# Maboroshi0327/MHAda-Style-Transfer

Hardware: AMD Instinct MI355X
Metric: stylized frames/sec (whole job) at 512x512 batch 8 fp32 [configs[1]] (higher is better)
Workload: dtype f32; 1 GPU; stylize 512x512 content+style, batch 8; resolution=512, batch_per_gpu=8, global_batch=8, compute_dtype=f32, parallelism=replicas x1

## Files before the change

mhada-style-transfer_amd/csrc/abi.hip:

```cpp
#include "common.h"

#include <mutex>
#include <stdlib.h>
#include <string.h>

namespace mhada {

static thread_local std::string g_last_error;

void set_error(const std::string& msg) { g_last_error = msg; }

int fail(const std::string& msg) {
  set_error(msg);
  return MHADA_ERR_ARG;
}

int check_launch(const char* what) {
  const hipError_t e = hipGetLastError();
  if (e != hipSuccess) {
    set_error(std::string(what) + ": " + hipGetErrorString(e));
    return MHADA_ERR_LAUNCH;
  }
  return MHADA_OK;
}

namespace {
struct Knob {
  const char* name;
  int Tuning::*field;
};
const Knob kKnobs[] = {
    {"attn_fixed_shift", &Tuning::attn_fixed_shift}, {"attn_waves", &Tuning::attn_waves},
    {"attn_tk", &Tuning::attn_tk},                   {"attn_prio", &Tuning::attn_prio},
    {"vit_attn_vec", &Tuning::vit_attn_vec},         {"out3_mfma", &Tuning::out3_mfma},
    {"out3_tile", &Tuning::out3_tile},               {"gemm_pp", &Tuning::gemm_pp},
    {"gemm_persist", &Tuning::gemm_persist},         {"gemm_pp128", &Tuning::gemm_pp128},
    {"gemm_ldsepi", &Tuning::gemm_ldsepi},           {"gemm_n64", &Tuning::gemm_n64},
    {"conv_c64", &Tuning::conv_c64},                 {"conv_dir", &Tuning::conv_dir},                 {"gemm_rinit", &Tuning::gemm_rinit},
    {"tn_skinny_lds", &Tuning::tn_skinny_lds},       {"train_dkv_dma", &Tuning::train_dkv_dma},
    {"wino_split3", &Tuning::wino_split3},           {"gemm_s3_order", &Tuning::gemm_s3_order},
    {"wino4", &Tuning::wino4},                       {"upsample_quad", &Tuning::upsample_quad},
    {"xknob", &Tuning::xknob},
};

Tuning g_tuning;
std::once_flag g_tuning_once;

void read_env_once() {
  std::call_once(g_tuning_once, [] {
    for (const Knob& k : kKnobs) {
      std::string env = "MHADA_";
      for (const char* c = k.name; *c; ++c) env += (char)(*c >= 'a' && *c <= 'z' ? *c - 32 : *c);
      if (const char* v = getenv(env.c_str())) g_tuning.*k.field = atoi(v);
    }
  });
}

bool valid(const char* name, int v) {
  if (!strcmp(name, "attn_waves")) return v == 0 || v == 4 || v == 8;
  if (!strcmp(name, "attn_tk")) return v == 64 || v == 128;
  if (!strcmp(name, "gemm_n64")) return v == 128 || v == 256;
  if (!strcmp(name, "xknob")) return v >= 0 && v < 16;
  return v == 0 || v == 1;
}
}

const Tuning& tuning() {
  read_env_once();
  return g_tuning;
}

}

extern "C" int mhada_abi_version(void) { return 18; }

extern "C" const char* mhada_last_error(void) { return mhada::g_last_error.c_str(); }

extern "C" int mhada_set_tuning(const char* name, int value) {
  using namespace mhada;
  read_env_once();
  if (!name) return fail("mhada_set_tuning: null name");
  for (const Knob& k : kKnobs) {
    if (!strcmp(k.name, name)) {
      if (!valid(name, value)) return fail(std::string("mhada_set_tuning: bad value for ") + name);
      g_tuning.*k.field = value;
      return MHADA_OK;
    }
  }
  return fail(std::string("mhada_set_tuning: unknown knob ") + name);
}

extern "C" int mhada_get_tuning(const char* name, int* value) {
  using namespace mhada;
  read_env_once();
  if (!name || !value) return fail("mhada_get_tuning: null argument");
  for (const Knob& k : kKnobs) {
    if (!strcmp(k.name, name)) {
      *value = g_tuning.*k.field;
      return MHADA_OK;
    }
  }
  return fail(std::string("mhada_get_tuning: unknown knob ") + name);
}
```

mhada-style-transfer_amd/csrc/common.h:

```cpp
#pragma once
#include <hip/hip_runtime.h>
#include <stdint.h>
#include <string>

#include "../../include/mhada_hip.h"

typedef __bf16 bf16;
typedef __bf16 bf16x8 __attribute__((ext_vector_type(8)));
typedef __bf16 bf16x4 __attribute__((ext_vector_type(4)));
typedef float f32x16 __attribute__((ext_vector_type(16)));
typedef float f32x4 __attribute__((ext_vector_type(4)));
typedef float f32x2 __attribute__((ext_vector_type(2)));

#define MHADA_DEV __device__ __forceinline__

namespace mhada {

void set_error(const std::string& msg);
int fail(const std::string& msg);
int check_launch(const char* what);

struct Tuning {
  int attn_fixed_shift = 1;
  int attn_waves = 0;
  int attn_tk = 128;
  int attn_prio = 1;
  int vit_attn_vec = 1;
  int out3_mfma = 1;
  int out3_tile = 1;
  int gemm_pp = 1;
  int gemm_persist = 1;
  int gemm_pp128 = 1;
  int gemm_ldsepi = 1;
  int gemm_n64 = 128;
  int conv_c64 = 1;
  int conv_dir = 1;
  int gemm_rinit = 1;
  int tn_skinny_lds = 1;
  int wino4 = 1;
  int wino_split3 = 1;
  int gemm_s3_order = 1;
  int train_dkv_dma = 1;
  int upsample_quad = 1;
  int xknob = 0;
};
const Tuning& tuning();

int conv3x3_c64(const void* x, const void* w, const float* bias, void* y, int B, int H, int W, bool up, int relu,
                hipStream_t s);
int conv3x3_dir(const void* x, const void* w, const float* bias, void* y, int B, int H, int W, int cin, int cout,
                int relu, hipStream_t s);

int vit_batch_attn_hd(const void* qkv, void* out, int dtype, int L, int ntok, int heads, int head_dim, hipStream_t s);

template <typename T> MHADA_DEV float to_f32(T x);
template <> MHADA_DEV float to_f32<float>(float x) { return x; }
template <> MHADA_DEV float to_f32<bf16>(bf16 x) { return (float)x; }

template <typename T> MHADA_DEV T from_f32(float x);
template <> MHADA_DEV float from_f32<float>(float x) { return x; }
template <> MHADA_DEV bf16 from_f32<bf16>(float x) { return (bf16)x; }

template <typename T> struct Vec16;
template <> struct Vec16<float> { typedef f32x4 type; static constexpr int N = 4; };
template <> struct Vec16<bf16> { typedef bf16x8 type; static constexpr int N = 8; };

MHADA_DEV float bilerp(float ly0, float ly1, float lx0, float lx1, float x00, float x01, float x10, float x11) {
  return fmaf(ly1, fmaf(lx0, x10, lx1 * x11), ly0 * fmaf(lx0, x00, lx1 * x01));
}

MHADA_DEV float wave_sum(float v) {
#pragma unroll
  for (int o = 32; o > 0; o >>= 1) v += __shfl_xor(v, o, 64);
  return v;
}
MHADA_DEV float wave_max(float v) {
#pragma unroll
  for (int o = 32; o > 0; o >>= 1) v = fmaxf(v, __shfl_xor(v, o, 64));
  return v;
}

MHADA_DEV int xcd_remap(int bid, int nblk) {
  const int q = nblk / 8, r = nblk % 8;
  const int xcd = bid % 8, k = bid / 8;
  return (xcd < r ? xcd * (q + 1) : r * (q + 1) + (xcd - r) * q) + k;
}

}
```

mhada-style-transfer_amd/csrc/wino.hip:

```cpp
#include "common.h"

#include <algorithm>
#include <utility>

#ifndef WINO_DBG
#define WINO_DBG 0
#endif
#ifndef WINO4_DBG
#define WINO4_DBG 0
#endif

namespace mhada {

namespace {
constexpr int kT = 8;
constexpr int kTT = kT * kT;
constexpr int kCO = 64;
constexpr int kCK = 8;
constexpr int kRP = 2 * kT + 2;
constexpr int kRaw = kRP * kRP;
constexpr int kRDma = (2 * kRaw + 63) / 64;
constexpr int kVS = 16 * kTT * kCK;
constexpr int kUS = 16 * kCO * kCK;
constexpr int kRS = kRDma * 64 * 4;

struct WinoP {
  const float* x;
  const float* u;
  const float* bias;
  float* y;
  const float* mask;
  int B, H, W, Cin, Cout, Ho, Wo, pad, zero, relu;
  long long ldc;
  int nbx, nby, nbn, nblk;
};

MHADA_DEV int reflect_clamp(int v, int n) {
  v = v < 0 ? -v : (v >= n ? 2 * n - 2 - v : v);
  return min(max(v, 0), n - 1);
}
MHADA_DEV int swz(int row, int half) { return row * 8 + ((half ^ ((row >> 3) & 1)) << 2); }
MHADA_DEV int rswz(int slot) { return slot ^ (((slot >> 3) & 1) << 1); }
MHADA_DEV int rswz4(int slot) { return slot ^ (((slot >> 4) & 1) << 1); }
MHADA_DEV void glds16(const float* src, float* lds) {
  __builtin_amdgcn_global_load_lds((const __attribute__((address_space(1))) void*)src,
                                   (__attribute__((address_space(3))) void*)lds, 16, 0, 0);
}


__global__ void __launch_bounds__(512, 1) wino_kernel(const WinoP p) {
  __shared__ __attribute__((aligned(16))) float lds[2 * (kVS + kUS + kRS)];
  auto sV = [&](int i) { return lds + i * kVS; };
  auto sU = [&](int i) { return lds + 2 * kVS + i * kUS; };
  auto sR = [&](int i) { return lds + 2 * (kVS + kUS) + i * kRS; };
  const int tid = threadIdx.x, lane = tid & 63, h = lane >> 5, r32 = lane & 31;
  const int wave = __builtin_amdgcn_readfirstlane(tid >> 6);
  const int e = wave >> 2, th = wave & 1, ch = (wave >> 1) & 1;

  int id = xcd_remap(blockIdx.x, p.nblk);
  const int nb = id % p.nbn;
  id /= p.nbn;
  const int bx = id % p.nbx;
  id /= p.nbx;
  const int by = id % p.nby;
  const int b = id / p.nby;
  const int co0 = nb * kCO;
  const int P = p.zero ? p.pad : 1;
  const int nck = p.Cin / kCK;

  int roff[2];
#pragma unroll
  for (int t = 0; t < 2; ++t) {
    const int slot = rswz(64 * (wave + 8 * t) + lane);
    const int px = min(slot >> 1, kRaw - 1);
    int iy = 2 * by * kT - P + px / kRP, ix = 2 * bx * kT - P + px % kRP;
    if (p.zero) {
      iy = min(max(iy, 0), p.H - 1);
      ix = min(max(ix, 0), p.W - 1);
    } else {
      iy = reflect_clamp(iy, p.H);
      ix = reflect_clamp(ix, p.W);
    }
    roff[t] = ((b * p.H + iy) * p.W + ix) * p.Cin + 4 * (slot & 1);
  }
  int uoff[4];
#pragma unroll
  for (int t = 0; t < 4; ++t) {
    const int slot = 64 * (4 * wave + t) + lane;
    const int xi = slot >> 7, row = (slot >> 1) & 63, sh = slot & 1;
    uoff[t] = (xi * p.Cout + co0 + row) * kCK + 4 * (sh ^ ((row >> 3) & 1));
  }
  const long long ustride = (long long)16 * p.Cout * kCK;
  auto dma = [&](int cu, float* su, int cr, float* sr) {
#if WINO_DBG & 2
    return;
#endif
    cu = min(cu, nck - 1);
    cr = min(cr, nck - 1);
    const float* uc = p.u + cu * ustride;
#pragma unroll
    for (int t = 0; t < 4; ++t) glds16(uc + uoff[t], su + (4 * wave + t) * 256);
    glds16(p.x + roff[0] + cr * kCK, sr + wave * 256);
    if (wave + 8 < kRDma) glds16(p.x + roff[1] + cr * kCK, sr + (wave + 8) * 256);
  };
  const int tc = tid & 7, tt = tid >> 3;
  int roffs[16];
#pragma unroll
  for (int i = 0; i < 4; ++i)
#pragma unroll
    for (int j = 0; j < 4; ++j) {
      const int pix = (2 * (tt >> 3) + i) * kRP + 2 * (tt & 7) + j;
      roffs[4 * i + j] = rswz(2 * pix + (tc >> 2)) * 4 + (tc & 3);
    }
  const int vdst = swz(tt, tc >> 2) + (tc & 3);
  unsigned zmask = 0;
  if (p.zero) {
    const int y0 = 2 * (by * kT + (tt >> 3)) - P, x0 = 2 * (bx * kT + (tt & 7)) - P;
#pragma unroll
    for (int i = 0; i < 4; ++i)
#pragma unroll
      for (int j = 0; j < 4; ++j)
        if (y0 + i < 0 || y0 + i >= p.H || x0 + j < 0 || x0 + j >= p.W) zmask |= 1u << (4 * i + j);
  }
  auto transform = [&](const float* sr, float* sv) {
#if WINO_DBG & 4
    return;
#endif
    float d[16];
#pragma unroll
    for (int i = 0; i < 4; ++i)
#pragma unroll
      for (int j = 0; j < 4; ++j) {
        const float v = sr[roffs[4 * i + j]];
        d[4 * i + j] = (zmask >> (4 * i + j)) & 1 ? 0.f : v;
      }
    float t[16];
#pragma unroll
    for (int j = 0; j < 4; ++j) {
      t[0 * 4 + j] = d[0 * 4 + j] - d[2 * 4 + j];
      t[1 * 4 + j] = d[1 * 4 + j] + d[2 * 4 + j];
      t[2 * 4 + j] = d[2 * 4 + j] - d[1 * 4 + j];
      t[3 * 4 + j] = d[1 * 4 + j] - d[3 * 4 + j];
    }
#pragma unroll
    for (int i = 0; i < 4; ++i) {
      sv[(4 * i + 0) * kTT * kCK + vdst] = t[4 * i + 0] - t[4 * i + 2];
      sv[(4 * i + 1) * kTT * kCK + vdst] = t[4 * i + 1] + t[4 * i + 2];
      sv[(4 * i + 2) * kTT * kCK + vdst] = t[4 * i + 2] - t[4 * i + 1];
      sv[(4 * i + 3) * kTT * kCK + vdst] = t[4 * i + 1] - t[4 * i + 3];
    }
  };

  f32x16 acc[8];
#pragma unroll
  for (int x = 0; x < 8; ++x)
#pragma unroll
    for (int q = 0; q < 16; ++q) acc[x][q] = 0.f;
  const int arow = swz(32 * th + r32, h) + 8 * e * (kTT * kCK), brow = swz(32 * ch + r32, h) + 8 * e * (kCO * kCK);
  auto mfmas = [&](const float* sv, const float* su) {
#if WINO_DBG & 1
    return;
#endif
#pragma unroll
    for (int x = 0; x < 8; ++x) {
      const f32x4 av = *reinterpret_cast<const f32x4*>(sv + x * (kTT * kCK) + arow);
      const f32x4 bv = *reinterpret_cast<const f32x4*>(su + x * (kCO * kCK) + brow);
#pragma unroll
      for (int s = 0; s < 4; ++s) acc[x] = __builtin_amdgcn_mfma_f32_32x32x2f32(av[s], bv[s], acc[x], 0, 0, 0);
    }
  };
  auto publish = [&]() {
    __builtin_amdgcn_sched_barrier(0);
    asm volatile("s_waitcnt vmcnt(0)" ::: "memory");
    __syncthreads();
  };

  dma(0, sU(0), 0, sR(0));
  dma(0, sU(0), 1, sR(1));
  publish();
  transform(sR(0), sV(0));
  __syncthreads();
  for (int k = 0; k < nck; ++k) {
    const int c = k & 1, n = c ^ 1;
    dma(k + 1, sU(n), k + 2, sR(c));
    mfmas(sV(c), sU(c));
    transform(sR(n), sV(n));
    publish();
  }

  float* ex = lds + (wave & 3) * (16 * 4 * 64) + lane;
  static_assert(4 * 16 * 4 * 64 <= 2 * kVS, "epilogue exchange must fit sV");
  if (e) {
#pragma unroll
    for (int r = 0; r < 16; ++r) {
      float m[2][2];
#pragma unroll
      for (int i = 0; i < 2; ++i) {
        const float m0 = acc[4 * i][r], m1 = acc[4 * i + 1][r], m2 = acc[4 * i + 2][r], m3 = acc[4 * i + 3][r];
        m[i][0] = m0 + m1 + m2;
        m[i][1] = m1 - m2 - m3;
      }
#pragma unroll
      for (int q = 0; q < 2; ++q) {
        ex[(r * 4 + 2 * q) * 64] = m[0][q];
        ex[(r * 4 + 2 * q + 1) * 64] = -m[0][q] - m[1][q];
      }
    }
  }
  __syncthreads();
  if (e) return;
  const int co = co0 + 32 * ch + r32;
  const float bias = p.bias ? p.bias[co] : 0.f;
#pragma unroll
  for (int r = 0; r < 16; ++r) {
    const int tile = 32 * th + (r & 3) + 8 * (r >> 2) + 4 * h;
    float m[2][2];
#pragma unroll
    for (int i = 0; i < 2; ++i) {
      const float m0 = acc[4 * i][r], m1 = acc[4 * i + 1][r], m2 = acc[4 * i + 2][r], m3 = acc[4 * i + 3][r];
      m[i][0] = m0 + m1 + m2;
      m[i][1] = m1 - m2 - m3;
    }
    const int oy0 = 2 * (by * kT + (tile >> 3)), ox0 = 2 * (bx * kT + (tile & 7));
#pragma unroll
    for (int q = 0; q < 2; ++q) {
      float y0 = m[0][q] + m[1][q] + ex[(r * 4 + 2 * q) * 64] + bias;
      float y1 = m[1][q] + ex[(r * 4 + 2 * q + 1) * 64] + bias;
      if (p.relu) {
        y0 = fmaxf(y0, 0.f);
        y1 = fmaxf(y1, 0.f);
      }
      const int ox = ox0 + q;
      if (ox < p.Wo) {
        const long long i0 = ((long long)(b * p.Ho + oy0) * p.Wo + ox) * p.ldc + co;
        const long long i1 = i0 + (long long)p.Wo * p.ldc;
        if (p.mask) {
          if (oy0 < p.Ho && !(p.mask[i0] > 0.f)) y0 = 0.f;
          if (oy0 + 1 < p.Ho && !(p.mask[i1] > 0.f)) y1 = 0.f;
        }
        if (oy0 < p.Ho) p.y[i0] = y0;
        if (oy0 + 1 < p.Ho) p.y[i1] = y1;
      }
    }
  }
}

template <int DBG>
__global__ void __launch_bounds__(256, 1) wino4_kernel(const WinoP p) {
  __shared__ __attribute__((aligned(16))) float lds[2 * (kVS + kUS + kRS)];
  const int tid = threadIdx.x, lane = tid & 63, h = lane >> 5, r32 = lane & 31;
  const int wave = __builtin_amdgcn_readfirstlane(tid >> 6);
  const int th = wave & 1, ch = wave >> 1;

  int id = xcd_remap(blockIdx.x, p.nblk);
  const int nb = id % p.nbn;
  id /= p.nbn;
  const int bx = id % p.nbx;
  id /= p.nbx;
  const int by = id % p.nby;
  const int b = id / p.nby;
  const int co0 = nb * kCO;
  const int P = p.zero ? p.pad : 1;
  const int nck = p.Cin / kCK;

  const __amdgpu_buffer_rsrc_t xr = __builtin_amdgcn_make_buffer_rsrc(
      const_cast<float*>(p.x), 0, (int)((long long)p.B * p.H * p.W * p.Cin * 4), 0x00020000);
  const __amdgpu_buffer_rsrc_t ur =
      __builtin_amdgcn_make_buffer_rsrc(const_cast<float*>(p.u), 0, p.Cin * 16 * p.Cout * 4, 0x00020000);
  int rvo[3];
#pragma unroll
  for (int t = 0; t < 3; ++t) {
    const int slot = rswz4(64 * min(wave + 4 * t, kRDma - 1) + lane);
    const int px = min(slot >> 1, kRaw - 1);
    int iy = 2 * by * kT - P + px / kRP, ix = 2 * bx * kT - P + px % kRP;
    bool inside = true;
    if (p.zero) {
      inside = iy >= 0 && iy < p.H && ix >= 0 && ix < p.W;
    } else {
      iy = reflect_clamp(iy, p.H);
      ix = reflect_clamp(ix, p.W);
    }
    rvo[t] = inside ? (((b * p.H + iy) * p.W + ix) * p.Cin + 4 * (slot & 1)) * 4 : 0x7ff00000;
  }
  const bool raw2 = wave + 8 < kRDma;
  int uvo[8];
#pragma unroll
  for (int t = 0; t < 8; ++t) {
    const int slot = 64 * (8 * wave + t) + lane;
    const int xi = slot >> 7, row = (slot >> 1) & 63, sh = slot & 1;
    uvo[t] = ((xi * p.Cout + co0 + row) * kCK + 4 * (sh ^ ((row >> 3) & 1))) * 4;
  }
  const int ucb = 16 * p.Cout * kCK * 4;
  typedef __attribute__((address_space(3))) void* LdsP;
  auto dma_piece = [&](int i, int cu, int su, int cr, int sr) {
    if constexpr ((DBG & 1) != 0) return;
    if (i < 8) {
      float* dst = lds + 2 * kVS + su * kUS + (8 * wave + i) * 256;
      __builtin_amdgcn_raw_ptr_buffer_load_lds(ur, (LdsP)dst, 16, uvo[i], min(cu, nck - 1) * ucb, 0, 0);
    } else if (i < 10 || raw2) {
      float* dst = lds + 2 * (kVS + kUS) + sr * kRS + (wave + 4 * (i - 8)) * 256;
      __builtin_amdgcn_raw_ptr_buffer_load_lds(xr, (LdsP)dst, 16, rvo[i - 8], min(cr, nck - 1) * kCK * 4, 0, 0);
    }
  };
  const int tp = tid & 3, tt = tid >> 2;
  int roffs[16];
#pragma unroll
  for (int i = 0; i < 4; ++i)
#pragma unroll
    for (int j = 0; j < 4; ++j) {
      const int pix = (2 * (tt >> 3) + i) * kRP + 2 * (tt & 7) + j;
      roffs[4 * i + j] = (2 * (kVS + kUS) + rswz4(2 * pix + (tp >> 1)) * 4 + 2 * (tp & 1)) & 0xffff;
    }
  const int vdst = (swz(tt, tp >> 1) + 2 * (tp & 1)) & 0x7fff;
  f32x2 d[16], tv[16];
  auto tload = [&](int rbuf) {
    if constexpr ((DBG & 2) != 0) return;
#pragma unroll
    for (int q = 0; q < 16; ++q) d[q] = *reinterpret_cast<const f32x2*>(lds + roffs[q] + rbuf * kRS);
  };
  auto tcols = [&]() {
    if constexpr ((DBG & 2) != 0) return;
#pragma unroll
    for (int j = 0; j < 4; ++j) {
      tv[0 * 4 + j] = d[0 * 4 + j] - d[2 * 4 + j];
      tv[1 * 4 + j] = d[1 * 4 + j] + d[2 * 4 + j];
      tv[2 * 4 + j] = d[2 * 4 + j] - d[1 * 4 + j];
      tv[3 * 4 + j] = d[1 * 4 + j] - d[3 * 4 + j];
    }
  };
  auto trows = [&](int vbuf, int i0) {
    if constexpr ((DBG & 2) != 0) return;
#pragma unroll
    for (int i = i0; i < i0 + 2; ++i) {
      float* o = lds + vbuf * kVS + vdst;
      *reinterpret_cast<f32x2*>(o + (4 * i + 0) * kTT * kCK) = tv[4 * i + 0] - tv[4 * i + 2];
      *reinterpret_cast<f32x2*>(o + (4 * i + 1) * kTT * kCK) = tv[4 * i + 1] + tv[4 * i + 2];
      *reinterpret_cast<f32x2*>(o + (4 * i + 2) * kTT * kCK) = tv[4 * i + 2] - tv[4 * i + 1];
      *reinterpret_cast<f32x2*>(o + (4 * i + 3) * kTT * kCK) = tv[4 * i + 1] - tv[4 * i + 3];
    }
  };

  f32x16 acc[16];
#pragma unroll
  for (int x = 0; x < 16; ++x)
#pragma unroll
    for (int q = 0; q < 16; ++q) acc[x][q] = 0.f;
  const int arow = swz(32 * th + r32, h) & 0x7fff, brow = (2 * kVS + swz(32 * ch + r32, h)) & 0xffff;
  f32x4 oa[3], ob[3];
  auto rdop = [&](int xi, int buf, f32x4& a, f32x4& bb) {
    a = *reinterpret_cast<const f32x4*>(lds + buf * kVS + xi * (kTT * kCK) + arow);
    bb = *reinterpret_cast<const f32x4*>(lds + buf * kUS + xi * (kCO * kCK) + brow);
  };
  auto publish = [&]() {
    __builtin_amdgcn_sched_barrier(0);
    if constexpr ((DBG & 8) == 0) asm volatile("s_waitcnt vmcnt(0)" ::: "memory");
    __syncthreads();
  };
  auto fence = [&]() { __builtin_amdgcn_sched_barrier(0); };

#pragma unroll
  for (int i = 0; i < 11; ++i) dma_piece(i, 0, 0, 0, 0);
#pragma unroll
  for (int i = 8; i < 11; ++i) dma_piece(i, 0, 0, 1, 1);
  publish();
  tload(0);
  tcols();
  trows(0, 0);
  trows(0, 2);
  __syncthreads();
  auto chunk = [&](int k, auto cc) {
    constexpr int C = decltype(cc)::value, N = C ^ 1;
    rdop(0, C, oa[0], ob[0]);
    rdop(1, C, oa[1], ob[1]);
    fence();
#pragma unroll
    for (int xi = 0; xi < 16; ++xi) {
      if (xi + 2 < 16) rdop(xi + 2, C, oa[(xi + 2) % 3], ob[(xi + 2) % 3]);
      if constexpr ((DBG & 4) == 0) {
#pragma unroll
        for (int s = 0; s < 4; ++s)
          acc[xi] = __builtin_amdgcn_mfma_f32_32x32x2f32(oa[xi % 3][s], ob[xi % 3][s], acc[xi], 0, 0, 0);
      }
      if (xi < 11) dma_piece(xi, k + 1, N, k + 2, C);
      if (xi == 2) tload(N);
      if (xi == 4) { tcols(); trows(N, 0); }
      if (xi == 5) trows(N, 2);
      fence();
    }
    publish();
  };
  int k = 0;
  for (; k + 1 < nck; k += 2) {
    chunk(k, std::integral_constant<int, 0>());
    chunk(k + 1, std::integral_constant<int, 1>());
  }
  if (k < nck) chunk(k, std::integral_constant<int, 0>());

  const int co = co0 + 32 * ch + r32;
  const float bias = p.bias ? p.bias[co] : 0.f;
#pragma unroll
  for (int r = 0; r < 16; ++r) {
    const int tile = 32 * th + (r & 3) + 8 * (r >> 2) + 4 * h;
    float m[4][2];
#pragma unroll
    for (int i = 0; i < 4; ++i) {
      const float m0 = acc[4 * i][r], m1 = acc[4 * i + 1][r], m2 = acc[4 * i + 2][r], m3 = acc[4 * i + 3][r];
      m[i][0] = m0 + m1 + m2;
      m[i][1] = m1 - m2 - m3;
    }
    const int oy0 = 2 * (by * kT + (tile >> 3)), ox0 = 2 * (bx * kT + (tile & 7));
#pragma unroll
    for (int q = 0; q < 2; ++q) {
      const float e1 = -m[2][q] - m[3][q];
      float y0 = m[0][q] + m[1][q] + m[2][q] + bias;
      float y1 = m[1][q] + e1 + bias;
      if (p.relu) {
        y0 = fmaxf(y0, 0.f);
        y1 = fmaxf(y1, 0.f);
      }
      const int ox = ox0 + q;
      if (ox < p.Wo) {
        const long long i0 = ((long long)(b * p.Ho + oy0) * p.Wo + ox) * p.ldc + co;
        const long long i1 = i0 + (long long)p.Wo * p.ldc;
        if (p.mask) {
          if (oy0 < p.Ho && !(p.mask[i0] > 0.f)) y0 = 0.f;
          if (oy0 + 1 < p.Ho && !(p.mask[i1] > 0.f)) y1 = 0.f;
        }
        if (oy0 < p.Ho) p.y[i0] = y0;
        if (oy0 + 1 < p.Ho) p.y[i1] = y1;
      }
    }
  }
}

constexpr int kSK = 16;
constexpr int kSImg = 64 * kSK * 2;
constexpr int kSStage = 12 * kSImg;
constexpr int kSRDma = (4 * kRaw + 63) / 64;
constexpr int kSRawB = kSRDma * 1024;

struct WinoS3P : WinoP {
  const bf16* up;
};

MHADA_DEV int rpix(int pix) { return pix ^ ((pix >> 2) & 1); }

__global__ void __launch_bounds__(256, 1) wino_s3_kernel(const WinoS3P p) {
  __shared__ __attribute__((aligned(16))) unsigned char sV0[kSStage];
  __shared__ __attribute__((aligned(16))) unsigned char sV1[kSStage];
  __shared__ __attribute__((aligned(16))) unsigned char sU0[kSStage];
  __shared__ __attribute__((aligned(16))) unsigned char sU1[kSStage];
  __shared__ __attribute__((aligned(16))) unsigned char sR0[kSRawB];
  __shared__ __attribute__((aligned(16))) unsigned char sR1[kSRawB];
  const int tid = threadIdx.x, lane = tid & 63, h = lane >> 5, r32 = lane & 31;
  const int wave = __builtin_amdgcn_readfirstlane(tid >> 6);
  const int th = wave & 1, ch = wave >> 1;

  int id = xcd_remap(blockIdx.x, p.nblk);
  const int nsp = p.nblk / p.nbn;
  const int nb = id / nsp;
  id -= nb * nsp;
  const int bx = id % p.nbx;
  id /= p.nbx;
  const int by = id % p.nby;
  const int b = id / p.nby;
  const int co0 = nb * kCO;
  const int P = p.zero ? p.pad : 1;
  const int nck = p.Cin / kSK, nst = 4 * nck;

  const __amdgpu_buffer_rsrc_t xr = __builtin_amdgcn_make_buffer_rsrc(
      const_cast<float*>(p.x), 0, (int)((long long)p.B * p.H * p.W * p.Cin * 4), 0x00020000);
  const __amdgpu_buffer_rsrc_t ur =
      __builtin_amdgcn_make_buffer_rsrc(const_cast<bf16*>(p.up), 0, p.Cin * p.Cout * 96, 0x00020000);
  int rvo[6];
#pragma unroll
  for (int t = 0; t < 6; ++t) {
    const int slot = 64 * (wave + 4 * t) + lane;
    const int pix = rpix(slot >> 2);
    int iy = 2 * by * kT - P + pix / kRP, ix = 2 * bx * kT - P + pix % kRP;
    bool inside = pix < kRaw;
    if (p.zero) {
      inside = inside && iy >= 0 && iy < p.H && ix >= 0 && ix < p.W;
    } else {
      iy = reflect_clamp(iy, p.H);
      ix = reflect_clamp(ix, p.W);
    }
    rvo[t] = inside ? (((b * p.H + iy) * p.W + ix) * p.Cin + 4 * (slot & 3)) * 4 : 0x7ff00000;
  }
  int uvo[6];
#pragma unroll
  for (int t = 0; t < 6; ++t) {
    const int slot = 64 * (6 * wave + t) + lane;
    const int g = slot >> 7, row = (slot >> 1) & 63, sh = slot & 1;
    uvo[t] = ((g * p.Cout + co0 + row) * kSK + 8 * (sh ^ ((row >> 3) & 1))) * 2;
  }
  const int usb = 12 * p.Cout * kSK * 2;
  typedef __attribute__((address_space(3))) void* LdsP;

  const int tq = tid & 3, tt = tid >> 2;
  int roffs[16];
#pragma unroll
  for (int i = 0; i < 4; ++i)
#pragma unroll
    for (int j = 0; j < 4; ++j) roffs[4 * i + j] = rpix((2 * (tt >> 3) + i) * kRP + 2 * (tt & 7) + j) * 64 + tq * 16;
  const int vdst = tt * 32 + ((((tq >> 1) ^ (tt >> 3)) & 1) << 4) + (tq & 1) * 8;
  auto transform = [&](auto ic, const unsigned char* sr, unsigned char* sv) {
    constexpr int I = decltype(ic)::value;
    constexpr int RA = I == 0 ? 0 : (I == 2 ? 2 : 1), RB = I == 0 ? 2 : (I == 1 ? 2 : (I == 2 ? 1 : 3));
    f32x4 t[4];
#pragma unroll
    for (int j = 0; j < 4; ++j) {
      const f32x4 a = *reinterpret_cast<const f32x4*>(sr + roffs[4 * RA + j]);
      const f32x4 c = *reinterpret_cast<const f32x4*>(sr + roffs[4 * RB + j]);
      t[j] = I == 1 ? a + c : a - c;
    }
    const f32x4 v[4] = {t[0] - t[2], t[1] + t[2], t[2] - t[1], t[1] - t[3]};
#pragma unroll
    for (int x = 0; x < 4; ++x) {
      bf16x4 p0, p1, p2;
#pragma unroll
      for (int e = 0; e < 4; ++e) {
        const bf16 a = (bf16)v[x][e];
        const float r = v[x][e] - (float)a;
        const bf16 c = (bf16)r;
        p0[e] = a;
        p1[e] = c;
        p2[e] = (bf16)(r - (float)c);
      }
      *reinterpret_cast<bf16x4*>(sv + (3 * x + 0) * kSImg + vdst) = p0;
      *reinterpret_cast<bf16x4*>(sv + (3 * x + 1) * kSImg + vdst) = p1;
      *reinterpret_cast<bf16x4*>(sv + (3 * x + 2) * kSImg + vdst) = p2;
    }
  };

  f32x16 acc[16];
#pragma unroll
  for (int x = 0; x < 16; ++x)
#pragma unroll
    for (int q = 0; q < 16; ++q) acc[x][q] = 0.f;
  const int fsw = (h ^ ((r32 >> 3) & 1)) << 4;
  const int aoff = (32 * th + r32) * 32 + fsw, boff = (32 * ch + r32) * 32 + fsw;
  auto mfmas = [&](auto ic, const unsigned char* sv, const unsigned char* su) {
    constexpr int I = decltype(ic)::value;
    constexpr int TA[6] = {1, 2, 0, 1, 0, 0}, TB[6] = {1, 0, 2, 0, 1, 0};
#pragma unroll
    for (int pr = 0; pr < 2; ++pr) {
      bf16x8 a[2][3], bq[2][3];
#pragma unroll
      for (int x = 0; x < 2; ++x)
#pragma unroll
        for (int pl = 0; pl < 3; ++pl) {
          a[x][pl] = *reinterpret_cast<const bf16x8*>(sv + (3 * (2 * pr + x) + pl) * kSImg + aoff);
          bq[x][pl] = *reinterpret_cast<const bf16x8*>(su + (3 * (2 * pr + x) + pl) * kSImg + boff);
        }
#pragma unroll
      for (int t = 0; t < 6; ++t)
#pragma unroll
        for (int x = 0; x < 2; ++x)
          acc[4 * I + 2 * pr + x] =
              __builtin_amdgcn_mfma_f32_32x32x16_bf16(a[x][TA[t]], bq[x][TB[t]], acc[4 * I + 2 * pr + x], 0, 0, 0);
    }
  };
  auto publish = [&]() {
    __builtin_amdgcn_sched_barrier(0);
    asm volatile("s_waitcnt vmcnt(0)" ::: "memory");
    __syncthreads();
  };
  auto dma_u = [&](int s, unsigned char* su) {
    const int so = min(s, nst - 1) * usb;
#pragma unroll
    for (int t = 0; t < 6; ++t)
      __builtin_amdgcn_raw_ptr_buffer_load_lds(ur, (LdsP)(su + (6 * wave + t) * 1024), 16, (unsigned)uvo[t], so, 0, 0);
  };
  auto dma_raw = [&](int t0, int k, unsigned char* sr) {
    const int so = min(k, nck - 1) * kSK * 4;
#pragma unroll
    for (int t = t0; t < t0 + 3; ++t)
      if (t < 5 || wave == 0)
        __builtin_amdgcn_raw_ptr_buffer_load_lds(xr, (LdsP)(sr + (wave + 4 * t) * 1024), 16, (unsigned)rvo[t], so, 0, 0);
  };

  dma_u(0, sU0);
  dma_raw(0, 0, sR0);
  dma_raw(3, 0, sR0);
  publish();
  transform(std::integral_constant<int, 0>(), sR0, sV0);
  __syncthreads();
  auto stage = [&](int k, auto ic, auto cc) {
    constexpr int I = decltype(ic)::value, C = decltype(cc)::value;
    unsigned char* const svn = (I & 1) ? sV0 : sV1;
    dma_u(4 * k + I + 1, (I & 1) ? sU0 : sU1);
    if constexpr (I < 2) dma_raw(3 * I, k + 1, C ? sR0 : sR1);
    __builtin_amdgcn_sched_barrier(0);
    if constexpr (I < 3)
      transform(std::integral_constant<int, I + 1>(), C ? sR1 : sR0, svn);
    else
      transform(std::integral_constant<int, 0>(), C ? sR0 : sR1, svn);
    mfmas(ic, (I & 1) ? sV1 : sV0, (I & 1) ? sU1 : sU0);
    publish();
  };
  auto chunk = [&](int k, auto cc) {
    stage(k, std::integral_constant<int, 0>(), cc);
    stage(k, std::integral_constant<int, 1>(), cc);
    stage(k, std::integral_constant<int, 2>(), cc);
    stage(k, std::integral_constant<int, 3>(), cc);
  };
  int k = 0;
  for (; k + 1 < nck; k += 2) {
    chunk(k, std::integral_constant<int, 0>());
    chunk(k + 1, std::integral_constant<int, 1>());
  }
  if (k < nck) chunk(k, std::integral_constant<int, 0>());

  const int co = co0 + 32 * ch + r32;
  const float bias = p.bias ? p.bias[co] : 0.f;
#pragma unroll
  for (int r = 0; r < 16; ++r) {
    const int tile = 32 * th + (r & 3) + 8 * (r >> 2) + 4 * h;
    float m[4][2];
#pragma unroll
    for (int i = 0; i < 4; ++i) {
      const float m0 = acc[4 * i][r], m1 = acc[4 * i + 1][r], m2 = acc[4 * i + 2][r], m3 = acc[4 * i + 3][r];
      m[i][0] = m0 + m1 + m2;
      m[i][1] = m1 - m2 - m3;
    }
    const int oy0 = 2 * (by * kT + (tile >> 3)), ox0 = 2 * (bx * kT + (tile & 7));
#pragma unroll
    for (int q = 0; q < 2; ++q) {
      const float e1 = -m[2][q] - m[3][q];
      float y0 = m[0][q] + m[1][q] + m[2][q] + bias;
      float y1 = m[1][q] + e1 + bias;
      if (p.relu) {
        y0 = fmaxf(y0, 0.f);
        y1 = fmaxf(y1, 0.f);
      }
      const int ox = ox0 + q;
      if (ox < p.Wo) {
        const long long i0 = ((long long)(b * p.Ho + oy0) * p.Wo + ox) * p.ldc + co;
        const long long i1 = i0 + (long long)p.Wo * p.ldc;
        if (p.mask) {
          if (oy0 < p.Ho && !(p.mask[i0] > 0.f)) y0 = 0.f;
          if (oy0 + 1 < p.Ho && !(p.mask[i1] > 0.f)) y1 = 0.f;
        }
        if (oy0 < p.Ho) p.y[i0] = y0;
        if (oy0 + 1 < p.Ho) p.y[i1] = y1;
      }
    }
  }
}

__global__ void wino_weights_s3_kernel(const float* __restrict__ w, bf16* __restrict__ up, int Cout, int Cin) {
  const long long i = (long long)blockIdx.x * blockDim.x + threadIdx.x;
  if (i >= (long long)Cout * Cin) return;
  const int ci = (int)(i % Cin), co = (int)(i / Cin);
  float g[9];
#pragma unroll
  for (int t = 0; t < 9; ++t) g[t] = w[((long long)co * 9 + t) * Cin + ci];
  float gg[12];
#pragma unroll
  for (int kx = 0; kx < 3; ++kx) {
    const float a = g[kx], bb = g[3 + kx], c = g[6 + kx];
    gg[0 * 3 + kx] = a;
    gg[1 * 3 + kx] = 0.5f * (a + bb + c);
    gg[2 * 3 + kx] = 0.5f * (a - bb + c);
    gg[3 * 3 + kx] = c;
  }
  bf16* ub = up + ((long long)(ci / kSK) * 48 * Cout + co) * kSK + (ci % kSK);
#pragma unroll
  for (int r = 0; r < 4; ++r) {
    const float a = gg[3 * r], bb = gg[3 * r + 1], c = gg[3 * r + 2];
    const float v[4] = {a, 0.5f * (a + bb + c), 0.5f * (a - bb + c), c};
#pragma unroll
    for (int j = 0; j < 4; ++j) {
      const bf16 p0 = (bf16)v[j];
      const float r1 = v[j] - (float)p0;
      const bf16 p1 = (bf16)r1;
      bf16* o = ub + (long long)(4 * r + j) * 3 * Cout * kSK;
      o[0] = p0;
      o[(long long)Cout * kSK] = p1;
      o[2LL * Cout * kSK] = (bf16)(r1 - (float)p1);
    }
  }
}

__global__ void wino_weights_kernel(const float* __restrict__ w, float* __restrict__ u, int Cout, int Cin) {
  const long long i = (long long)blockIdx.x * blockDim.x + threadIdx.x;
  if (i >= (long long)Cout * Cin) return;
  const int ci = (int)(i % Cin), co = (int)(i / Cin);
  float g[9];
#pragma unroll
  for (int t = 0; t < 9; ++t) g[t] = w[((long long)co * 9 + t) * Cin + ci];
  float gg[12];
#pragma unroll
  for (int kx = 0; kx < 3; ++kx) {
    const float a = g[kx], bb = g[3 + kx], c = g[6 + kx];
    gg[0 * 3 + kx] = a;
    gg[1 * 3 + kx] = 0.5f * (a + bb + c);
    gg[2 * 3 + kx] = 0.5f * (a - bb + c);
    gg[3 * 3 + kx] = c;
  }
  float* ub = u + ((long long)(ci / kCK) * 16 * Cout + co) * kCK + (ci % kCK);
#pragma unroll
  for (int r = 0; r < 4; ++r) {
    const float a = gg[3 * r], bb = gg[3 * r + 1], c = gg[3 * r + 2];
    const float v[4] = {a, 0.5f * (a + bb + c), 0.5f * (a - bb + c), c};
#pragma unroll
    for (int j = 0; j < 4; ++j) ub[(long long)(4 * r + j) * Cout * kCK] = v[j];
  }
}
constexpr int kWgT = 8;
constexpr int kWgS = 16 * 64 * kWgT;
constexpr int kWgRX = 4 * 18 * 64;
constexpr int kWgRY = 2 * 16 * 64;

struct WgP {
  const float* x;
  const float* g;
  float* slab;
  float* cslab;
  int B, H, W, Cin, Cout, zero;
  long long ldg;
  int crow, nchunk, cps;
};

MHADA_DEV int wg_px(int px, int c) { return px * 64 + (c ^ (8 * ((px >> 1) & 7))); }

template <bool ZERO>
__global__ void __launch_bounds__(512, 1) wino_wgrad_kernel(const WgP p) {
  __shared__ __attribute__((aligned(16))) float lds[4 * kWgS + kWgRX + kWgRY];
  auto sYh = [&](int i) { return lds + i * kWgS; };
  auto sVb = [&](int i) { return lds + (2 + i) * kWgS; };
  float* sRX = lds + 4 * kWgS;
  float* sRY = sRX + kWgRX;
  const int tid = threadIdx.x, lane = tid & 63, h = lane >> 5, r32 = lane & 31;
  const int wave = __builtin_amdgcn_readfirstlane(tid >> 6);
  const int e = wave >> 2, coh = wave & 1, cih = (wave >> 1) & 1;
  const int nib = p.Cin / 64;
  const int cb = blockIdx.x / nib, ib = blockIdx.x - cb * nib;
  const int co0 = cb * 64, ci0 = ib * 64;
  const int c_beg = blockIdx.y * p.cps, c_end = min(p.nchunk, c_beg + p.cps);
  constexpr int P = 1;
  const int TW = p.crow * kWgT, TH = p.H / 2;

  struct Pos { int b, ty, tx0; };
  auto step_pos = [&](Pos& q) {
    q.tx0 += kWgT;
    if (q.tx0 >= TW) {
      q.tx0 = 0;
      if (++q.ty >= TH) {
        q.ty = 0;
        ++q.b;
      }
    }
  };
  auto src_pix = [&](int b, int Y, int X) -> long long {
    if (ZERO) {
      Y = min(max(Y, 0), p.H - 1);
      X = min(max(X, 0), p.W - 1);
    } else {
      Y = reflect_clamp(Y, p.H);
      X = reflect_clamp(X, p.W);
    }
    return ((long long)b * p.H + Y) * p.W + X;
  };
  const int ypx = 4 * wave + (lane >> 4), ysq = (lane & 15) ^ (2 * ((ypx >> 1) & 7));
  const long long yoff = ((long long)(ypx >> 4) * p.W + (ypx & 15)) * p.ldg + 4 * ysq;
  int xpx[3], xsq[3];
  long long xoff[3];
#pragma unroll
  for (int j = 0; j < 3; ++j) {
    xpx[j] = 4 * (wave + 8 * j) + (lane >> 4);
    xsq[j] = (lane & 15) ^ (2 * ((xpx[j] >> 1) & 7));
    xoff[j] = ((long long)(xpx[j] / 18) * p.W + xpx[j] % 18) * p.Cin + 4 * xsq[j];
  }
  auto interior = [&](const Pos& q) {
    return q.ty > 0 && 2 * q.ty + 2 < p.H && q.tx0 > 0 && 2 * q.tx0 + 16 < p.W;
  };
  auto dma = [&](const Pos& q) {
#if WINO_DBG & 2
    return;
#endif
    glds16(p.g + (((long long)q.b * p.H + 2 * q.ty) * p.W + 2 * q.tx0) * p.ldg + co0 + yoff, sRY + wave * 256);
    if (interior(q)) {
      const float* xb = p.x + (((long long)q.b * p.H + 2 * q.ty - P) * p.W + 2 * q.tx0 - P) * p.Cin + ci0;
#pragma unroll
      for (int j = 0; j < 3; ++j)
        if (wave + 8 * j < 18) glds16(xb + xoff[j], sRX + (wave + 8 * j) * 256);
    } else {
#pragma unroll
      for (int j = 0; j < 3; ++j)
        if (wave + 8 * j < 18) {
          const long long pix = src_pix(q.b, 2 * q.ty - P + xpx[j] / 18, 2 * q.tx0 - P + xpx[j] % 18);
          glds16(p.x + pix * p.Cin + ci0 + 4 * xsq[j], sRX + (wave + 8 * j) * 256);
        }
    }
  };
  const int it = lane & 7, irow = 8 * wave + (lane >> 3);
  const int wdst = swz(irow, it >> 2) + (it & 3);
  int ry[4], rx[16];
#pragma unroll
  for (int i = 0; i < 2; ++i)
#pragma unroll
    for (int j = 0; j < 2; ++j) ry[2 * i + j] = wg_px(16 * i + 2 * it + j, irow);
#pragma unroll
  for (int i = 0; i < 4; ++i)
#pragma unroll
    for (int j = 0; j < 4; ++j) rx[4 * i + j] = wg_px(18 * i + 2 * it + j, irow);
  float bsum = 0.f;
  auto transform = [&](const Pos& q, int n) {
#if WINO_DBG & 4
    return;
#endif
    float d[2][2];
#pragma unroll
    for (int i = 0; i < 2; ++i)
#pragma unroll
      for (int j = 0; j < 2; ++j) d[i][j] = sRY[ry[2 * i + j]];
    if (ib == 0) bsum += (d[0][0] + d[0][1]) + (d[1][0] + d[1][1]);
    float a[4][2];
#pragma unroll
    for (int j = 0; j < 2; ++j) {
      a[0][j] = d[0][j];
      a[1][j] = d[0][j] + d[1][j];
      a[2][j] = d[0][j] - d[1][j];
      a[3][j] = -d[1][j];
    }
    float* yh = sYh(n);
#pragma unroll
    for (int i = 0; i < 4; ++i) {
      yh[(4 * i + 0) * 512 + wdst] = a[i][0];
      yh[(4 * i + 1) * 512 + wdst] = a[i][0] + a[i][1];
      yh[(4 * i + 2) * 512 + wdst] = a[i][0] - a[i][1];
      yh[(4 * i + 3) * 512 + wdst] = -a[i][1];
    }
    float v[16];
#pragma unroll
    for (int i = 0; i < 16; ++i) v[i] = sRX[rx[i]];
    if (ZERO && !interior(q)) {
#pragma unroll
      for (int i = 0; i < 4; ++i)
#pragma unroll
        for (int j = 0; j < 4; ++j) {
          const int Y = 2 * q.ty - P + i, X = 2 * q.tx0 - P + 2 * it + j;
          if (Y < 0 || Y >= p.H || X < 0 || X >= p.W) v[4 * i + j] = 0.f;
        }
    }
    float t[16];
#pragma unroll
    for (int j = 0; j < 4; ++j) {
      t[0 * 4 + j] = v[0 * 4 + j] - v[2 * 4 + j];
      t[1 * 4 + j] = v[1 * 4 + j] + v[2 * 4 + j];
      t[2 * 4 + j] = v[2 * 4 + j] - v[1 * 4 + j];
      t[3 * 4 + j] = v[1 * 4 + j] - v[3 * 4 + j];
    }
    float* sv = sVb(n);
#pragma unroll
    for (int i = 0; i < 4; ++i) {
      sv[(4 * i + 0) * 512 + wdst] = t[4 * i + 0] - t[4 * i + 2];
      sv[(4 * i + 1) * 512 + wdst] = t[4 * i + 1] + t[4 * i + 2];
      sv[(4 * i + 2) * 512 + wdst] = t[4 * i + 2] - t[4 * i + 1];
      sv[(4 * i + 3) * 512 + wdst] = t[4 * i + 1] - t[4 * i + 3];
    }
  };

  f32x16 acc[8];
#pragma unroll
  for (int x = 0; x < 8; ++x)
#pragma unroll
    for (int q = 0; q < 16; ++q) acc[x][q] = 0.f;
  const int arow = swz(32 * coh + r32, h) + 8 * e * 512, brow = swz(32 * cih + r32, h) + 8 * e * 512;
  auto mfmas = [&](int n) {
#if WINO_DBG & 1
    return;
#endif
#pragma unroll
    for (int x = 0; x < 8; ++x) {
      const f32x4 av = *reinterpret_cast<const f32x4*>(sYh(n) + x * 512 + arow);
      const f32x4 bv = *reinterpret_cast<const f32x4*>(sVb(n) + x * 512 + brow);
#pragma unroll
      for (int s = 0; s < 4; ++s) acc[x] = __builtin_amdgcn_mfma_f32_32x32x2f32(av[s], bv[s], acc[x], 0, 0, 0);
    }
  };
  auto publish = [&]() {
    __builtin_amdgcn_sched_barrier(0);
    asm volatile("s_waitcnt vmcnt(0)" ::: "memory");
    __syncthreads();
  };

  if (c_beg < c_end) {
    Pos q;
    {
      const int per_img = TH * p.crow;
      q.b = c_beg / per_img;
      const int r = c_beg - q.b * per_img;
      q.ty = r / p.crow;
      q.tx0 = (r - q.ty * p.crow) * kWgT;
    }
    dma(q);
    publish();
    transform(q, 0);
    __syncthreads();
    for (int c = c_beg; c < c_end; ++c) {
      const int k = c - c_beg, cur = k & 1;
      const bool more = c + 1 < c_end;
      step_pos(q);
      if (more) dma(q);
      mfmas(cur);
      if (more) {
        asm volatile("s_waitcnt vmcnt(0)" ::: "memory");
        __syncthreads();
        transform(q, cur ^ 1);
      }
      __syncthreads();
    }
  }
  float* sl = p.slab + (long long)blockIdx.y * 16 * p.Cout * p.Cin;
#pragma unroll
  for (int x = 0; x < 8; ++x)
#pragma unroll
    for (int r = 0; r < 16; ++r) {
      const int co = co0 + 32 * coh + (r & 3) + 8 * (r >> 2) + 4 * h, ci = ci0 + 32 * cih + r32;
      sl[((long long)(8 * e + x) * p.Cout + co) * p.Cin + ci] = acc[x][r];
    }
  if (p.cslab && ib == 0) {
    bsum += __shfl_xor(bsum, 1, 64);
    bsum += __shfl_xor(bsum, 2, 64);
    bsum += __shfl_xor(bsum, 4, 64);
    if (it == 0) p.cslab[(long long)blockIdx.y * p.Cout + co0 + irow] = bsum;
  }
}

__global__ void __launch_bounds__(256) wino_wgrad_finish_kernel(const float* __restrict__ slab,
                                                                const float* __restrict__ cslab, float* __restrict__ dw,
                                                                float* __restrict__ db, int Cout, int Cin, int S) {
  const long long i = (long long)blockIdx.x * 256 + threadIdx.x;
  if (i >= (long long)Cout * Cin) return;
  const int co = (int)(i / Cin), ci = (int)(i - (long long)co * Cin);
  const long long st = (long long)Cout * Cin;
  float u[16];
#pragma unroll
  for (int x = 0; x < 16; ++x) u[x] = 0.f;
  for (int s = 0; s < S; ++s) {
    const float* q = slab + (long long)s * 16 * st + i;
#pragma unroll
    for (int x = 0; x < 16; ++x) u[x] += q[x * st];
  }
  float m[3][4];
#pragma unroll
  for (int c = 0; c < 4; ++c) {
    m[0][c] = u[0 * 4 + c] + 0.5f * (u[1 * 4 + c] + u[2 * 4 + c]);
    m[1][c] = 0.5f * (u[1 * 4 + c] - u[2 * 4 + c]);
    m[2][c] = 0.5f * (u[1 * 4 + c] + u[2 * 4 + c]) + u[3 * 4 + c];
  }
  float* o = dw + (long long)co * 9 * Cin + ci;
#pragma unroll
  for (int a = 0; a < 3; ++a) {
    o[(3 * a + 0) * Cin] = m[a][0] + 0.5f * (m[a][1] + m[a][2]);
    o[(3 * a + 1) * Cin] = 0.5f * (m[a][1] - m[a][2]);
    o[(3 * a + 2) * Cin] = 0.5f * (m[a][1] + m[a][2]) + m[a][3];
  }
  if (db && cslab && ci == 0) {
    float sb = 0.f;
    for (int s = 0; s < S; ++s) sb += cslab[(long long)s * Cout + co];
    db[co] = sb;
  }
}
}

}

using namespace mhada;

extern "C" int mhada_conv3x3_wgrad_wino_splits(int B, int H, int W, int Cin, int Cout) {
  if (B <= 0 || H < 2 || W < 16 || Cin <= 0 || Cout <= 0 || Cin % 64 || Cout % 64) return 0;
  const long long nchunk = (long long)B * (H / 2) * (W / 16);
  const long long blocks = (long long)(Cout / 64) * (Cin / 64);
  const long long s = std::max<long long>(1, std::min<long long>((512 + blocks - 1) / blocks, nchunk / 16));
  return (int)std::min<long long>(s, 65535);
}

extern "C" int mhada_conv3x3_wgrad_wino(const float* x, const float* g, float* dw, float* db, float* work,
                                        long long work_floats, int B, int H, int W, int Cin, int Cout, long long ldg,
                                        int pad_mode, mhada_stream_t s_) {
  if (!x || !g || !dw || !work || B <= 0 || H < 2 || W < 2 || Cin <= 0 || Cout <= 0)
    return fail("mhada_conv3x3_wgrad_wino: bad args");
  if (Cin % 64 || Cout % 64 || H % 2 || W % 16)
    return fail("mhada_conv3x3_wgrad_wino: needs Cin % 64 == 0, Cout % 64 == 0, H even, W % 16 == 0");
  if (pad_mode != MHADA_PAD_REFLECT && pad_mode != MHADA_PAD_ZERO) return fail("mhada_conv3x3_wgrad_wino: bad pad_mode");
  if (ldg < Cout || ldg % 4) return fail("mhada_conv3x3_wgrad_wino: ldg >= Cout, ldg % 4 == 0");
  if (((uintptr_t)x | (uintptr_t)g | (uintptr_t)work) & 15) return fail("mhada_conv3x3_wgrad_wino: 16-byte aligned x, g, work");
  if ((long long)B * H * W * std::max<long long>(Cin, ldg) > (1LL << 31) - 1)
    return fail("mhada_conv3x3_wgrad_wino: problem too large for 32-bit indexing");
  WgP p;
  p.x = x; p.g = g;
  p.B = B; p.H = H; p.W = W; p.Cin = Cin; p.Cout = Cout; p.ldg = ldg;
  p.zero = pad_mode == MHADA_PAD_ZERO;
  p.crow = W / 16;
  p.nchunk = B * (H / 2) * p.crow;
  int S = mhada_conv3x3_wgrad_wino_splits(B, H, W, Cin, Cout);
  const long long per = 16LL * Cout * Cin + (db ? Cout : 0);
  S = (int)std::min<long long>(S, work_floats / per);
  if (S < 1) return fail("mhada_conv3x3_wgrad_wino: workspace smaller than 16*Cout*Cin (+Cout) floats");
  p.cps = (p.nchunk + S - 1) / S;
  S = (p.nchunk + p.cps - 1) / p.cps;
  p.slab = work;
  p.cslab = db ? work + (long long)S * 16 * Cout * Cin : nullptr;
  const dim3 grid((unsigned)((Cout / 64) * (Cin / 64)), (unsigned)S);
  if (p.zero)
    hipLaunchKernelGGL(wino_wgrad_kernel<true>, grid, dim3(512), 0, (hipStream_t)s_, p);
  else
    hipLaunchKernelGGL(wino_wgrad_kernel<false>, grid, dim3(512), 0, (hipStream_t)s_, p);
  if (int rc = check_launch("mhada_conv3x3_wgrad_wino")) return rc;
  const long long n = (long long)Cout * Cin;
  hipLaunchKernelGGL(wino_wgrad_finish_kernel, dim3((unsigned)((n + 255) / 256)), dim3(256), 0, (hipStream_t)s_,
                     p.slab, p.cslab, dw, db, Cout, Cin, S);
  return check_launch("mhada_conv3x3_wgrad_wino(finish)");
}

extern "C" int mhada_wino_weights(const float* w, float* u, int Cout, int Cin, mhada_stream_t s_) {
  if (!w || !u || Cout <= 0 || Cin <= 0 || Cin % kCK) return fail("mhada_wino_weights: bad args (Cin % 8 == 0)");
  const long long n = (long long)Cout * Cin;
  hipLaunchKernelGGL(wino_weights_kernel, dim3((unsigned)((n + 255) / 256)), dim3(256), 0, (hipStream_t)s_, w, u,
                     Cout, Cin);
  return check_launch("mhada_wino_weights");
}

static int conv3x3_wino_launch(const float* x, const float* u, const void* up, const float* bias, float* y, int B,
                               int H, int W, int Cin, int Cout, long long ldc, int pad_mode, int pad, int relu,
                               const float* relu_mask, mhada_stream_t s_) {
  if (!x || !u || !y || B <= 0 || H < 2 || W < 2 || Cin <= 0 || Cout <= 0)
    return fail("mhada_conv3x3_wino: bad args");
  if (Cin % kCK || Cout % kCO) return fail("mhada_conv3x3_wino: needs Cin % 8 == 0 and Cout % 64 == 0");
  if (pad_mode != MHADA_PAD_REFLECT && pad_mode != MHADA_PAD_ZERO) return fail("mhada_conv3x3_wino: bad pad_mode");
  if (pad_mode == MHADA_PAD_ZERO && pad != 1 && pad != 2) return fail("mhada_conv3x3_wino: zero pad must be 1 or 2");
  if (ldc < Cout) return fail("mhada_conv3x3_wino: ldc < Cout");
  if (((uintptr_t)x | (uintptr_t)u) & 15) return fail("mhada_conv3x3_wino: x and u must be 16-byte aligned");
  WinoP p;
  p.x = x; p.u = u; p.bias = bias; p.y = y; p.mask = relu_mask;
  p.B = B; p.H = H; p.W = W; p.Cin = Cin; p.Cout = Cout;
  p.zero = pad_mode == MHADA_PAD_ZERO;
  p.pad = p.zero ? pad : 1;
  p.Ho = p.zero ? H + 2 * (pad - 1) : H;
  p.Wo = p.zero ? W + 2 * (pad - 1) : W;
  p.relu = relu;
  p.ldc = ldc;
  const int TY = (p.Ho + 1) / 2, TX = (p.Wo + 1) / 2;
  p.nby = (TY + kT - 1) / kT;
  p.nbx = (TX + kT - 1) / kT;
  p.nbn = Cout / kCO;
  const long long nblk = (long long)B * p.nby * p.nbx * p.nbn;
  if (nblk > (1LL << 31) - 1 || (long long)B * H * W * Cin > (1LL << 31) - 1)
    return fail("mhada_conv3x3_wino: problem too large for 32-bit indexing");
  p.nblk = (int)nblk;
  const bool bufx = (long long)B * H * W * Cin * 4 < 0x7ff00000LL;
  if (up && tuning().wino_split3 && Cin % kSK == 0 && bufx && (long long)Cin * Cout * 96 < 0x7ff00000LL) {
    if ((uintptr_t)up & 15) return fail("mhada_conv3x3_wino_split3: up must be 16-byte aligned");
    WinoS3P q;
    static_cast<WinoP&>(q) = p;
    q.up = (const bf16*)up;
    hipLaunchKernelGGL(wino_s3_kernel, dim3(p.nblk), dim3(256), 0, (hipStream_t)s_, q);
  } else if (tuning().wino4 && bufx) {
    hipLaunchKernelGGL(wino4_kernel<WINO4_DBG>, dim3(p.nblk), dim3(256), 0, (hipStream_t)s_, p);
  } else
    hipLaunchKernelGGL(wino_kernel, dim3(p.nblk), dim3(512), 0, (hipStream_t)s_, p);
  return check_launch("mhada_conv3x3_wino");
}

extern "C" int mhada_conv3x3_wino(const float* x, const float* u, const float* bias, float* y, int B, int H, int W,
                                  int Cin, int Cout, long long ldc, int pad_mode, int pad, int relu,
                                  const float* relu_mask, mhada_stream_t s_) {
  return conv3x3_wino_launch(x, u, nullptr, bias, y, B, H, W, Cin, Cout, ldc, pad_mode, pad, relu, relu_mask, s_);
}

extern "C" int mhada_conv3x3_wino_split3(const float* x, const float* u, const void* up, const float* bias, float* y,
                                         int B, int H, int W, int Cin, int Cout, long long ldc, int pad_mode, int pad,
                                         int relu, const float* relu_mask, mhada_stream_t s_) {
  if (!up) return fail("mhada_conv3x3_wino_split3: bad args");
  return conv3x3_wino_launch(x, u, up, bias, y, B, H, W, Cin, Cout, ldc, pad_mode, pad, relu, relu_mask, s_);
}

extern "C" int mhada_wino_weights_split3(const float* w, void* up, int Cout, int Cin, mhada_stream_t s_) {
  if (!w || !up || Cout <= 0 || Cin <= 0 || Cin % kSK) return fail("mhada_wino_weights_split3: bad args (Cin % 16 == 0)");
  const long long n = (long long)Cout * Cin;
  hipLaunchKernelGGL(wino_weights_s3_kernel, dim3((unsigned)((n + 255) / 256)), dim3(256), 0, (hipStream_t)s_, w,
                     (bf16*)up, Cout, Cin);
  return check_launch("mhada_wino_weights_split3");
}
```

Measured before the change: 342.7 frames/s.

## Prefetch raw input two chunks ahead in split3 Winograd kernel with partial waitcnt

Adds a ring-prefetch variant of the split3 Winograd conv kernel. Raw-input DMA for chunk k+2 is issued early, and each stage's barrier waits with vmcnt(2) or vmcnt(3) instead of draining all outstanding loads. The aim is to hide global-to-LDS load latency behind the transform and MFMA work instead of stalling at every stage. It relies on exact vmcnt accounting, so any mismatch in load ordering could cause races. The variant is gated by a new knob that defaults on, and debug template flags for skipping work are added.

```diff
diff --git a/mhada-style-transfer_amd/csrc/abi.hip b/mhada-style-transfer_amd/csrc/abi.hip
--- a/mhada-style-transfer_amd/csrc/abi.hip
+++ b/mhada-style-transfer_amd/csrc/abi.hip
@@ -40,7 +40,7 @@
     {"tn_skinny_lds", &Tuning::tn_skinny_lds},       {"train_dkv_dma", &Tuning::train_dkv_dma},
     {"wino_split3", &Tuning::wino_split3},           {"gemm_s3_order", &Tuning::gemm_s3_order},
     {"wino4", &Tuning::wino4},                       {"upsample_quad", &Tuning::upsample_quad},
-    {"xknob", &Tuning::xknob},
+    {"wino_s3_ring", &Tuning::wino_s3_ring},         {"xknob", &Tuning::xknob},
 };
 
 Tuning g_tuning;
diff --git a/mhada-style-transfer_amd/csrc/common.h b/mhada-style-transfer_amd/csrc/common.h
--- a/mhada-style-transfer_amd/csrc/common.h
+++ b/mhada-style-transfer_amd/csrc/common.h
@@ -39,6 +39,7 @@
   int tn_skinny_lds = 1;
   int wino4 = 1;
   int wino_split3 = 1;
+  int wino_s3_ring = 1;
   int gemm_s3_order = 1;
   int train_dkv_dma = 1;
   int upsample_quad = 1;
diff --git a/mhada-style-transfer_amd/csrc/wino.hip b/mhada-style-transfer_amd/csrc/wino.hip
--- a/mhada-style-transfer_amd/csrc/wino.hip
+++ b/mhada-style-transfer_amd/csrc/wino.hip
@@ -8,6 +8,9 @@
 #endif
 #ifndef WINO4_DBG
 #define WINO4_DBG 0
+#endif
+#ifndef WINO_S3_DBG
+#define WINO_S3_DBG 0
 #endif
 
 namespace mhada {
@@ -445,6 +448,7 @@
 
 MHADA_DEV int rpix(int pix) { return pix ^ ((pix >> 2) & 1); }
 
+template <int DBG, int RING>
 __global__ void __launch_bounds__(256, 1) wino_s3_kernel(const WinoS3P p) {
   __shared__ __attribute__((aligned(16))) unsigned char sV0[kSStage];
   __shared__ __attribute__((aligned(16))) unsigned char sV1[kSStage];
@@ -566,13 +570,24 @@
     asm volatile("s_waitcnt vmcnt(0)" ::: "memory");
     __syncthreads();
   };
+  auto publish_ring = [&](auto kc) {
+    constexpr int keep = decltype(kc)::value;
+    __builtin_amdgcn_sched_barrier(0);
+    if constexpr (keep == 3) asm volatile("s_waitcnt vmcnt(3) lgkmcnt(0)" ::: "memory");
+    else if constexpr (keep == 2) asm volatile("s_waitcnt vmcnt(2) lgkmcnt(0)" ::: "memory");
+    else asm volatile("s_waitcnt vmcnt(0) lgkmcnt(0)" ::: "memory");
+    __builtin_amdgcn_s_barrier();
+    __builtin_amdgcn_sched_barrier(0);
+  };
   auto dma_u = [&](int s, unsigned char* su) {
+    if constexpr (DBG & 1) return;
     const int so = min(s, nst - 1) * usb;
 #pragma unroll
     for (int t = 0; t < 6; ++t)
       __builtin_amdgcn_raw_ptr_buffer_load_lds(ur, (LdsP)(su + (6 * wave + t) * 1024), 16, (unsigned)uvo[t], so, 0, 0);
   };
   auto dma_raw = [&](int t0, int k, unsigned char* sr) {
+    if constexpr (DBG & 2) return;
     const int so = min(k, nck - 1) * kSK * 4;
 #pragma unroll
     for (int t = t0; t < t0 + 3; ++t)
@@ -584,20 +599,37 @@
   dma_raw(0, 0, sR0);
   dma_raw(3, 0, sR0);
   publish();
-  transform(std::integral_constant<int, 0>(), sR0, sV0);
-  __syncthreads();
+  if constexpr (RING) {
+    dma_raw(0, 1, sR1);
+    __builtin_amdgcn_sched_barrier(0);
+  }
+  if constexpr ((DBG & 4) == 0) transform(std::integral_constant<int, 0>(), sR0, sV0);
+  if constexpr (RING)
+    publish_ring(std::integral_constant<int, 3>());
+  else
+    __syncthreads();
   auto stage = [&](int k, auto ic, auto cc) {
     constexpr int I = decltype(ic)::value, C = decltype(cc)::value;
     unsigned char* const svn = (I & 1) ? sV0 : sV1;
     dma_u(4 * k + I + 1, (I & 1) ? sU0 : sU1);
-    if constexpr (I < 2) dma_raw(3 * I, k + 1, C ? sR0 : sR1);
+    if constexpr (RING) {
+      if constexpr (I == 3) dma_raw(0, k + 2, C ? sR1 : sR0);
+      if constexpr (I == 0) dma_raw(3, k + 1, C ? sR0 : sR1);
+    } else {
+      if constexpr (I < 2) dma_raw(3 * I, k + 1, C ? sR0 : sR1);
+    }
     __builtin_amdgcn_sched_barrier(0);
-    if constexpr (I < 3)
-      transform(std::integral_constant<int, I + 1>(), C ? sR1 : sR0, svn);
+    if constexpr ((DBG & 4) == 0) {
+      if constexpr (I < 3)
+        transform(std::integral_constant<int, I + 1>(), C ? sR1 : sR0, svn);
+      else
+        transform(std::integral_constant<int, 0>(), C ? sR0 : sR1, svn);
+    }
+    mfmas(ic, (I & 1) ? sV1 : sV0, (I & 1) ? sU1 : sU0);
+    if constexpr (RING)
+      publish_ring(std::integral_constant<int, I == 3 ? 3 : (I == 0 ? 2 : 0)>());
     else
-      transform(std::integral_constant<int, 0>(), C ? sR0 : sR1, svn);
-    mfmas(ic, (I & 1) ? sV1 : sV0, (I & 1) ? sU1 : sU0);
-    publish();
+      publish();
   };
   auto chunk = [&](int k, auto cc) {
     stage(k, std::integral_constant<int, 0>(), cc);
@@ -611,6 +643,7 @@
     chunk(k + 1, std::integral_constant<int, 1>());
   }
   if (k < nck) chunk(k, std::integral_constant<int, 0>());
+  if constexpr (RING) asm volatile("s_waitcnt vmcnt(0)" ::: "memory");
 
   const int co = co0 + 32 * ch + r32;
   const float bias = p.bias ? p.bias[co] : 0.f;
@@ -1058,7 +1091,10 @@
     WinoS3P q;
     static_cast<WinoP&>(q) = p;
     q.up = (const bf16*)up;
-    hipLaunchKernelGGL(wino_s3_kernel, dim3(p.nblk), dim3(256), 0, (hipStream_t)s_, q);
+    if (tuning().wino_s3_ring)
+      hipLaunchKernelGGL((wino_s3_kernel<WINO_S3_DBG, 1>), dim3(p.nblk), dim3(256), 0, (hipStream_t)s_, q);
+    else
+      hipLaunchKernelGGL((wino_s3_kernel<WINO_S3_DBG, 0>), dim3(p.nblk), dim3(256), 0, (hipStream_t)s_, q);
   } else if (tuning().wino4 && bufx) {
     hipLaunchKernelGGL(wino4_kernel<WINO4_DBG>, dim3(p.nblk), dim3(256), 0, (hipStream_t)s_, p);
   } else
```

After: 343.3 frames/s (median of 6 runs). About the same (+0.2%).
